# autonomousvision/LaRa

Hardware: AMD Instinct MI355X
Metric: novel-view frames/sec @512x512 (4-view in, 2DGS fwd+bwd) (higher is better)
Workload: dtype f32 raster + bf16-MFMA/f32-accumulate encoder (+ bf16-autocast coarse decoder MLP, as the reference's bf16-mixed)

## Files before the change

### lara_amd/csrc/group_attn.h

```cpp
#pragma once
#include "mfma_gemm.h"

namespace {


__device__ __forceinline__ float wave_total(float x) {
    x += dpp_move<0xB1, 0xf>(x);
    x += dpp_move<0x4E, 0xf>(x);
    x += dpp_move<0x141, 0xf>(x);
    x += dpp_move<0x140, 0xf>(x);
    x += dpp_move<0x142, 0xa>(x);
    x += dpp_move<0x143, 0xc>(x);
    return __int_as_float(__builtin_amdgcn_readlane(__float_as_int(x), 63));
}


__global__ void __launch_bounds__(256) pack_weight_frag_kernel(const unsigned short *__restrict__ W0, unsigned short *__restrict__ out0,
                                                               const unsigned short *__restrict__ W1, unsigned short *__restrict__ out1) {
    const bool second = blockIdx.x >= 32;
    const unsigned short *W = second ? W1 : W0;
    unsigned short *out = second ? out1 : out0;
    const int t = (blockIdx.x & 31) * 256 + threadIdx.x;
    const int lane = t & 63, ks = (t >> 6) & 15, nt = t >> 10;
    *(uint4 *)(out + (size_t)t * 8) = *(const uint4 *)(W + (size_t)(nt * 32 + (lane & 31)) * 256 + ks * 16 + 8 * (lane >> 5));
}

template <bool KEEP>
__global__ void __launch_bounds__(64)
group_attn_fused2_kernel(const float *x , const float *__restrict__ gamma,
                        const float *__restrict__ beta, const float eps, const unsigned short *__restrict__ Wq ,
                        const unsigned short *__restrict__ KV, const unsigned short *__restrict__ Wo , float *y, const int G,
                        unsigned short *__restrict__ xn_out, unsigned short *__restrict__ q_out, unsigned short *__restrict__ o_out) {
    constexpr int GA_LDS = 24576;
    __shared__ __attribute__((aligned(16))) unsigned char lds_all[GA_LDS];
    const int lane = threadIdx.x & 63;
    const int unit = blockIdx.x, g0 = unit * 4;
    if (g0 >= G) return;
    unsigned char *R = lds_all, *KVr = R + 16384;
    const int c16 = lane & 15, q4 = lane >> 4;
    const int q_rows = min(32, (G - g0) * 8), kv_rows = min(16, (G - g0) * 4);
    const int srow = lane >> 4, sphys = lane & 15;
    const size_t row0 = (size_t)g0 * 8;

    {
        const float4 gm = ((const float4 *)gamma)[lane], bt = ((const float4 *)beta)[lane];
        const int hh = lane >> 5, chunk = (lane & 31) >> 1, sub = (lane & 1) * 8;
#pragma unroll 1
        for (int rb = 0; rb < 32; rb += 16) {
            float4 v[16];
#pragma unroll
            for (int i = 0; i < 16; i++) v[i] = ((const float4 *)(x + (row0 + min(rb + i, q_rows - 1)) * 256))[lane];
#pragma unroll
            for (int i = 0; i < 16; i++) {
                const int r = rb + i;
                const float mean = wave_total((v[i].x + v[i].y) + (v[i].z + v[i].w)) * (1.0f / 256.0f);
                const float a = v[i].x - mean, b = v[i].y - mean, c = v[i].z - mean, d4 = v[i].w - mean;
                const float rstd = 1.0f / sqrtf(wave_total(a * a + b * b + c * c + d4 * d4) * (1.0f / 256.0f) + eps);
                *(uint2 *)(R + hh * 8192 + r * 256 + ((chunk ^ (r & 15)) << 4) + sub) =
                    make_uint2(f2bf2(a * rstd * gm.x + bt.x, b * rstd * gm.y + bt.y), f2bf2(c * rstd * gm.z + bt.z, d4 * rstd * gm.w + bt.w));
            }
        }
    }
    const int frow = lane & 31, fk = 8 * (lane >> 5);
    auto load_rows = [&](bf16x8 (&bf)[16]) {
#pragma unroll
        for (int ks = 0; ks < 16; ks++) {
            const int f = ks * 16 + fk;
            bf[ks] = *(const bf16x8 *)(R + (f >> 7) * 8192 + frow * 256 + ((((f & 127) >> 3) ^ (frow & 15)) << 4));
        }
    };
#pragma unroll
    for (int i = 0; i < 4; i++) {
        const int row = 4 * i + srow, chunk = sphys ^ (row & 15);
        const unsigned short *src = KV + (size_t)(g0 * 4 + min(row, kv_rows - 1)) * 512 + chunk * 8;
        __builtin_amdgcn_global_load_lds((const __attribute__((address_space(1))) void *)src,
                                         (__attribute__((address_space(3))) void *)(KVr + i * 1024), 16, 0, 0);
        __builtin_amdgcn_global_load_lds((const __attribute__((address_space(1))) void *)(src + 256),
                                         (__attribute__((address_space(3))) void *)(KVr + 4096 + i * 1024), 16, 0, 0);
    }
    auto store_rows = [&](unsigned short *dst) {
        asm volatile("s_waitcnt lgkmcnt(0)" ::: "memory");
#pragma unroll 4
        for (int i = 0; i < 16; i++) {
            const int r = 2 * i + (lane >> 5), c = lane & 31;
            const uint4 v = *(const uint4 *)(R + (c >> 4) * 8192 + r * 256 + (((c & 15) ^ (r & 15)) << 4));
            if (r < q_rows) *(uint4 *)(dst + (row0 + r) * 256 + c * 8) = v;
        }
    };
    bf16x8 bf[16], wf[16];
    load_rows(bf);
    if (KEEP) store_rows(xn_out);
#pragma unroll
    for (int ks = 0; ks < 16; ks++) wf[ks] = *(const bf16x8 *)(Wq + ((size_t)ks * 64 + lane) * 8);
#pragma unroll 1
    for (int nt = 0; nt < 8; nt++) {
        const unsigned short *wnext = Wq + ((size_t)min(nt + 1, 7) * 1024 + lane) * 8;
        bf16x8 wn[16];
#pragma unroll
        for (int ks = 0; ks < 16; ks++) wn[ks] = *(const bf16x8 *)(wnext + ks * 512);
        f32x16 acc;
#pragma unroll
        for (int i = 0; i < 16; i++) acc[i] = 0.f;
#pragma unroll
        for (int ks = 0; ks < 16; ks++) acc = __builtin_amdgcn_mfma_f32_32x32x16_bf16(wf[ks], bf[ks], acc, 0, 0, 0);
#pragma unroll
        for (int g = 0; g < 4; g++) {
            const int f = nt * 32 + 8 * g + 4 * (lane >> 5);
            *(uint2 *)(R + (f >> 7) * 8192 + frow * 256 + ((((f & 127) >> 3) ^ (frow & 15)) << 4) + ((f & 7) << 1)) =
                make_uint2(f2bf2(acc[4 * g], acc[4 * g + 1]), f2bf2(acc[4 * g + 2], acc[4 * g + 3]));
        }
#pragma unroll
        for (int ks = 0; ks < 16; ks++) wf[ks] = wn[ks];
    }
    if (KEEP) store_rows(q_out);
    asm volatile("s_waitcnt vmcnt(0)" ::: "memory");
    uint4 pk[4], pv[4];
#pragma unroll
    for (int i = 0; i < 4; i++) {
        const int row = 4 * i + srow, chunk = sphys ^ (row & 15);
        const unsigned short *src = KV + (size_t)(g0 * 4 + min(row, kv_rows - 1)) * 512 + 128 + chunk * 8;
        pk[i] = *(const uint4 *)src;
        pv[i] = *(const uint4 *)(src + 256);
    }
    for (int hh = 0; hh < 2; hh++) {
        unsigned char *Qr = R + hh * 8192, *Kr = KVr, *Vr = KVr + 4096;
        asm volatile("s_waitcnt lgkmcnt(0)" ::: "memory");
        if (hh == 1) {
#pragma unroll
            for (int i = 0; i < 4; i++) {
                *(uint4 *)(Kr + i * 1024 + lane * 16) = pk[i];
                *(uint4 *)(Vr + i * 1024 + lane * 16) = pv[i];
            }
            asm volatile("s_waitcnt lgkmcnt(0)" ::: "memory");
        }
#pragma unroll 2
        for (int hl = 0; hl < 8; hl++) {
            const int ck = 2 * hl + (q4 >> 1), sub = (q4 & 1) * 8;
            const s16x4 kf = *(const s16x4 *)(Kr + c16 * 256 + ((ck ^ c16) << 4) + sub);
            s16x4 vf;
            const int cv = 2 * hl + (c16 >> 3), vb = (c16 & 7) * 2;
#pragma unroll
            for (int e = 0; e < 4; e++) {
                const int row = 4 * q4 + e;
                vf[e] = *(const short *)(Vr + row * 256 + ((cv ^ row) << 4) + vb);
            }
#pragma unroll
            for (int t = 0; t < 2; t++) {
                const int qrow = 16 * t + c16;
                const s16x4 qf = *(const s16x4 *)(Qr + qrow * 256 + ((ck ^ (qrow & 15)) << 4) + sub);
                f32x4 sc = {0.f, 0.f, 0.f, 0.f};
                sc = __builtin_amdgcn_mfma_f32_16x16x16bf16_1k(kf, qf, sc, 0, 0, 0);
                const bool valid = q4 == 2 * t + (c16 >> 3);
                const float s0 = sc[0] * 0.25f, s1 = sc[1] * 0.25f, s2 = sc[2] * 0.25f, s3 = sc[3] * 0.25f;
                const float mx = fmaxf(fmaxf(s0, s1), fmaxf(s2, s3));
                const float e0 = __expf(s0 - mx), e1 = __expf(s1 - mx), e2 = __expf(s2 - mx), e3 = __expf(s3 - mx);
                const float inv = valid ? 1.0f / (e0 + e1 + e2 + e3) : 0.f;
                const uint2 pp = make_uint2(f2bf2(e0 * inv, e1 * inv), f2bf2(e2 * inv, e3 * inv));
                s16x4 pf;
                __builtin_memcpy(&pf, &pp, 8);
                f32x4 o = {0.f, 0.f, 0.f, 0.f};
                o = __builtin_amdgcn_mfma_f32_16x16x16bf16_1k(pf, vf, o, 0, 0, 0);
                const unsigned o01 = f2bf2(o[0], o[1]), o23 = f2bf2(o[2], o[3]);
#pragma unroll
                for (int rr = 0; rr < 4; rr++) {
                    const int orow = 16 * t + 4 * q4 + rr;
                    const unsigned w = rr < 2 ? o01 : o23;
                    *(unsigned short *)(Qr + orow * 256 + ((cv ^ (orow & 15)) << 4) + vb) = (unsigned short)((rr & 1) ? (w >> 16) : w);
                }
            }
        }
    }
    asm volatile("s_waitcnt lgkmcnt(0)" ::: "memory");
    if (KEEP) store_rows(o_out);
    load_rows(bf);
#pragma unroll
    for (int ks = 0; ks < 16; ks++) wf[ks] = *(const bf16x8 *)(Wo + ((size_t)ks * 64 + lane) * 8);
    float *T = (float *)R;
    const int erow = lane >> 3, ec = (lane & 7) * 4;
    float4 xr[4], xn4[4];
#pragma unroll
    for (int p4 = 0; p4 < 4; p4++) xr[p4] = *(const float4 *)(x + (row0 + min(erow + 8 * p4, q_rows - 1)) * 256 + ec);
#pragma unroll 1
    for (int nt = 0; nt < 8; nt++) {
        const unsigned short *wnext = Wo + ((size_t)min(nt + 1, 7) * 1024 + lane) * 8;
        bf16x8 wn[16];
#pragma unroll
        for (int ks = 0; ks < 16; ks++) wn[ks] = *(const bf16x8 *)(wnext + ks * 512);
#pragma unroll
        for (int p4 = 0; p4 < 4; p4++) xn4[p4] = *(const float4 *)(x + (row0 + min(erow + 8 * p4, q_rows - 1)) * 256 + min(nt + 1, 7) * 32 + ec);
        f32x16 acc;
#pragma unroll
        for (int i = 0; i < 16; i++) acc[i] = 0.f;
#pragma unroll
        for (int ks = 0; ks < 16; ks++) acc = __builtin_amdgcn_mfma_f32_32x32x16_bf16(wf[ks], bf[ks], acc, 0, 0, 0);
#pragma unroll
        for (int g = 0; g < 4; g++)
            *(float4 *)(T + frow * 36 + 8 * g + 4 * (lane >> 5)) = make_float4(acc[4 * g], acc[4 * g + 1], acc[4 * g + 2], acc[4 * g + 3]);
#pragma unroll
        for (int p4 = 0; p4 < 4; p4++) {
            const int row = erow + 8 * p4;
            const float4 v = *(const float4 *)(T + row * 36 + ec);
            if (row < q_rows)
                *(float4 *)(y + (row0 + row) * 256 + nt * 32 + ec) = make_float4(v.x + xr[p4].x, v.y + xr[p4].y, v.z + xr[p4].z, v.w + xr[p4].w);
        }
#pragma unroll
        for (int ks = 0; ks < 16; ks++) wf[ks] = wn[ks];
#pragma unroll
        for (int p4 = 0; p4 < 4; p4++) xr[p4] = xn4[p4];
    }
}

}
```

Baseline: 985.4.

## Split attention KV staging into quarter-heads to shrink LDS and raise occupancy

Restructures the fused group-attention kernel so K/V are staged into LDS one quarter (64 columns) at a time instead of per half, which cuts the LDS footprint from 24KB to 20KB. It also sets launch_bounds min-blocks to 2 and switches the intermediate xn/q/o stores to nontemporal stores. The goal is more resident waves per CU and less cache pollution, at the cost of more register prefetch of K/V (six fragments held) and four attend passes with extra waits. It also adds compile-time GA_TIMING switches that fake loads for profiling, plus a separate probe entry point.

After: 978.1. Within noise of the previous version (-0.7%).

```diff
diff --git a/lara_amd/csrc/attn_probe.hip b/lara_amd/csrc/attn_probe.hip
--- /dev/null
+++ b/lara_amd/csrc/attn_probe.hip
@@ -0,0 +1,27 @@
+#include "mfma_gemm.h"
+#include "group_attn.h"
+
+extern "C" {
+
+int lara_attnprobe_step(int keep, int project, int G, int cond_dim, const float *x, const unsigned short *cond_bf16, const float *ln_w,
+                        const float *ln_b, float eps, const unsigned short *wq, const unsigned short *wkv, const unsigned short *wo,
+                        float *y, unsigned short *kv, unsigned short *xn, unsigned short *q, unsigned short *o, void *wpack, void *stream) {
+    hipStream_t s = (hipStream_t)stream;
+    if (G <= 0 || !x || !ln_w || !ln_b || !wq || !wo || !y || !kv || !wpack) return hipErrorInvalidValue;
+    if (keep && (!xn || !q || !o)) return hipErrorInvalidValue;
+    if (project) {
+        if (!cond_bf16 || !wkv || cond_dim <= 0 || cond_dim % 32) return hipErrorInvalidValue;
+        GemmP p{};
+        p.A = cond_bf16; p.W = wkv; p.C = kv; p.M = G * 4; p.N = 512; p.K = cond_dim;
+        const hipError_t e = launch_gemm_ring<0, 0>(p, s);
+        if (e != hipSuccess) return e;
+    }
+    unsigned short *wqp = (unsigned short *)wpack, *wop = wqp + 65536;
+    const hipError_t e = L2D_LAUNCH_ERR(s, pack_weight_frag_kernel, dim3(64), dim3(256), 0, wq, wqp, wo, wop);
+    if (e != hipSuccess) return e;
+    if (keep) return L2D_LAUNCH_ERR(s, group_attn_fused2_kernel<true>, dim3((G + 3) / 4), dim3(64), 0, x, ln_w, ln_b, eps, wqp, kv, wop, y, G, xn, q, o);
+    return L2D_LAUNCH_ERR(s, group_attn_fused2_kernel<false>, dim3((G + 3) / 4), dim3(64), 0, x, ln_w, ln_b, eps, wqp, kv, wop, y, G,
+                          (unsigned short *)nullptr, (unsigned short *)nullptr, (unsigned short *)nullptr);
+}
+
+}
diff --git a/lara_amd/csrc/group_attn.h b/lara_amd/csrc/group_attn.h
--- a/lara_amd/csrc/group_attn.h
+++ b/lara_amd/csrc/group_attn.h
@@ -25,13 +25,17 @@
     *(uint4 *)(out + (size_t)t * 8) = *(const uint4 *)(W + (size_t)(nt * 32 + (lane & 31)) * 256 + ks * 16 + 8 * (lane >> 5));
 }
 
+#ifndef GA_TIMING
+#define GA_TIMING 0
+#endif
 template <bool KEEP>
-__global__ void __launch_bounds__(64)
+__global__ void __launch_bounds__(64, 2)
 group_attn_fused2_kernel(const float *x , const float *__restrict__ gamma,
                         const float *__restrict__ beta, const float eps, const unsigned short *__restrict__ Wq ,
                         const unsigned short *__restrict__ KV, const unsigned short *__restrict__ Wo , float *y, const int G,
                         unsigned short *__restrict__ xn_out, unsigned short *__restrict__ q_out, unsigned short *__restrict__ o_out) {
-    constexpr int GA_LDS = 24576;
+    typedef unsigned u32x4 __attribute__((ext_vector_type(4)));
+    constexpr int GA_LDS = 20480;
     __shared__ __attribute__((aligned(16))) unsigned char lds_all[GA_LDS];
     const int lane = threadIdx.x & 63;
     const int unit = blockIdx.x, g0 = unit * 4;
@@ -41,6 +45,12 @@
     const int q_rows = min(32, (G - g0) * 8), kv_rows = min(16, (G - g0) * 4);
     const int srow = lane >> 4, sphys = lane & 15;
     const size_t row0 = (size_t)g0 * 8;
+    constexpr bool KEPT = KEEP && !(GA_TIMING & 32);
+    auto kv_off = [](const int r, const int c) { return (r >> 1) * 256 + (((((r & 1) << 3) + c) ^ (r >> 1)) << 4); };
+    auto kv_src = [&](const int qd, const int i) {
+        const int rv = 4 * i + srow, C = sphys ^ rv, r = 2 * rv + (C >> 3);
+        return KV + (size_t)(g0 * 4 + min(r, kv_rows - 1)) * 512 + qd * 64 + (C & 7) * 8;
+    };
 
     {
         const float4 gm = ((const float4 *)gamma)[lane], bt = ((const float4 *)beta)[lane];
@@ -49,7 +59,15 @@
         for (int rb = 0; rb < 32; rb += 16) {
             float4 v[16];
 #pragma unroll
-            for (int i = 0; i < 16; i++) v[i] = ((const float4 *)(x + (row0 + min(rb + i, q_rows - 1)) * 256))[lane];
+            for (int i = 0; i < 16; i++) {
+                if (GA_TIMING & 1) {
+                    float4 t = make_float4((float)lane, (float)(lane >> 1), (float)(lane & 7), 1.f);
+                    asm volatile("" : "+v"(t.x), "+v"(t.y), "+v"(t.z), "+v"(t.w));
+                    v[i] = t;
+                } else {
+                    v[i] = ((const float4 *)(x + (row0 + min(rb + i, q_rows - 1)) * 256))[lane];
+                }
+            }
 #pragma unroll
             for (int i = 0; i < 16; i++) {
                 const int r = rb + i;
@@ -69,35 +87,46 @@
             bf[ks] = *(const bf16x8 *)(R + (f >> 7) * 8192 + frow * 256 + ((((f & 127) >> 3) ^ (frow & 15)) << 4));
         }
     };
-#pragma unroll
-    for (int i = 0; i < 4; i++) {
-        const int row = 4 * i + srow, chunk = sphys ^ (row & 15);
-        const unsigned short *src = KV + (size_t)(g0 * 4 + min(row, kv_rows - 1)) * 512 + chunk * 8;
-        __builtin_amdgcn_global_load_lds((const __attribute__((address_space(1))) void *)src,
-                                         (__attribute__((address_space(3))) void *)(KVr + i * 1024), 16, 0, 0);
-        __builtin_amdgcn_global_load_lds((const __attribute__((address_space(1))) void *)(src + 256),
-                                         (__attribute__((address_space(3))) void *)(KVr + 4096 + i * 1024), 16, 0, 0);
+    if (!(GA_TIMING & 4)) {
+#pragma unroll
+        for (int i = 0; i < 2; i++) {
+            const unsigned short *src = kv_src(0, i);
+            __builtin_amdgcn_global_load_lds((const __attribute__((address_space(1))) void *)src,
+                                             (__attribute__((address_space(3))) void *)(KVr + i * 1024), 16, 0, 0);
+            __builtin_amdgcn_global_load_lds((const __attribute__((address_space(1))) void *)(src + 256),
+                                             (__attribute__((address_space(3))) void *)(KVr + 2048 + i * 1024), 16, 0, 0);
+        }
     }
     auto store_rows = [&](unsigned short *dst) {
         asm volatile("s_waitcnt lgkmcnt(0)" ::: "memory");
 #pragma unroll 4
         for (int i = 0; i < 16; i++) {
             const int r = 2 * i + (lane >> 5), c = lane & 31;
-            const uint4 v = *(const uint4 *)(R + (c >> 4) * 8192 + r * 256 + (((c & 15) ^ (r & 15)) << 4));
-            if (r < q_rows) *(uint4 *)(dst + (row0 + r) * 256 + c * 8) = v;
-        }
-    };
+            const u32x4 v = *(const u32x4 *)(R + (c >> 4) * 8192 + r * 256 + (((c & 15) ^ (r & 15)) << 4));
+            if (r < q_rows) __builtin_nontemporal_store(v, (u32x4 *)(dst + (row0 + r) * 256 + c * 8));
+        }
+    };
+    auto wfrag = [&](const unsigned short *W, const int nt, const int ks, const bool fake) {
+        if (fake) {
+            const unsigned u = 0x3c003c00u + lane + ks;
+            const u32x4 t = {u, u + 1, u + 2, u + 3};
+            bf16x8 r;
+            __builtin_memcpy(&r, &t, 16);
+            return r;
+        }
+        return *(const bf16x8 *)(W + ((size_t)(nt * 16 + ks) * 64 + lane) * 8);
+    };
+    constexpr bool FQ = GA_TIMING & 2, FO = GA_TIMING & 8;
     bf16x8 bf[16], wf[16];
     load_rows(bf);
-    if (KEEP) store_rows(xn_out);
-#pragma unroll
-    for (int ks = 0; ks < 16; ks++) wf[ks] = *(const bf16x8 *)(Wq + ((size_t)ks * 64 + lane) * 8);
+    if (KEPT) store_rows(xn_out);
+#pragma unroll
+    for (int ks = 0; ks < 16; ks++) wf[ks] = wfrag(Wq, 0, ks, FQ);
 #pragma unroll 1
     for (int nt = 0; nt < 8; nt++) {
-        const unsigned short *wnext = Wq + ((size_t)min(nt + 1, 7) * 1024 + lane) * 8;
         bf16x8 wn[16];
 #pragma unroll
-        for (int ks = 0; ks < 16; ks++) wn[ks] = *(const bf16x8 *)(wnext + ks * 512);
+        for (int ks = 0; ks < 16; ks++) wn[ks] = wfrag(Wq, min(nt + 1, 7), ks, FQ);
         f32x16 acc;
 #pragma unroll
         for (int i = 0; i < 16; i++) acc[i] = 0.f;
@@ -112,37 +141,46 @@
 #pragma unroll
         for (int ks = 0; ks < 16; ks++) wf[ks] = wn[ks];
     }
-    if (KEEP) store_rows(q_out);
+    if (KEPT) store_rows(q_out);
     asm volatile("s_waitcnt vmcnt(0)" ::: "memory");
-    uint4 pk[4], pv[4];
-#pragma unroll
-    for (int i = 0; i < 4; i++) {
-        const int row = 4 * i + srow, chunk = sphys ^ (row & 15);
-        const unsigned short *src = KV + (size_t)(g0 * 4 + min(row, kv_rows - 1)) * 512 + 128 + chunk * 8;
-        pk[i] = *(const uint4 *)src;
-        pv[i] = *(const uint4 *)(src + 256);
-    }
-    for (int hh = 0; hh < 2; hh++) {
-        unsigned char *Qr = R + hh * 8192, *Kr = KVr, *Vr = KVr + 4096;
+    u32x4 pk[6], pv[6];
+#pragma unroll
+    for (int qd = 1; qd < 4; qd++) {
+#pragma unroll
+        for (int i = 0; i < 2; i++) {
+            if (GA_TIMING & 4) {
+                pk[2 * (qd - 1) + i] = u32x4{(unsigned)lane, (unsigned)qd, (unsigned)i, 0x3c003c00u};
+                pv[2 * (qd - 1) + i] = u32x4{(unsigned)lane, (unsigned)i, (unsigned)qd, 0x3c003c00u};
+            } else {
+                const unsigned short *src = kv_src(qd, i);
+                pk[2 * (qd - 1) + i] = *(const u32x4 *)src;
+                pv[2 * (qd - 1) + i] = *(const u32x4 *)(src + 256);
+            }
+        }
+    }
+    auto attend = [&](auto qdc) __attribute__((always_inline)) {
+        constexpr int qd = decltype(qdc)::value;
+        unsigned char *Qr = R + (qd >> 1) * 8192, *Kr = KVr, *Vr = KVr + 2048;
         asm volatile("s_waitcnt lgkmcnt(0)" ::: "memory");
-        if (hh == 1) {
-#pragma unroll
-            for (int i = 0; i < 4; i++) {
-                *(uint4 *)(Kr + i * 1024 + lane * 16) = pk[i];
-                *(uint4 *)(Vr + i * 1024 + lane * 16) = pv[i];
+        if constexpr (qd > 0) {
+#pragma unroll
+            for (int i = 0; i < 2; i++) {
+                *(u32x4 *)(Kr + i * 1024 + lane * 16) = pk[2 * (qd - 1) + i];
+                *(u32x4 *)(Vr + i * 1024 + lane * 16) = pv[2 * (qd - 1) + i];
             }
             asm volatile("s_waitcnt lgkmcnt(0)" ::: "memory");
         }
 #pragma unroll 2
-        for (int hl = 0; hl < 8; hl++) {
+        for (int hp = 0; hp < 4; hp++) {
+            const int hl = (qd & 1) * 4 + hp;
             const int ck = 2 * hl + (q4 >> 1), sub = (q4 & 1) * 8;
-            const s16x4 kf = *(const s16x4 *)(Kr + c16 * 256 + ((ck ^ c16) << 4) + sub);
+            const s16x4 kf = *(const s16x4 *)(Kr + kv_off(c16, 2 * hp + (q4 >> 1)) + sub);
             s16x4 vf;
             const int cv = 2 * hl + (c16 >> 3), vb = (c16 & 7) * 2;
 #pragma unroll
             for (int e = 0; e < 4; e++) {
                 const int row = 4 * q4 + e;
-                vf[e] = *(const short *)(Vr + row * 256 + ((cv ^ row) << 4) + vb);
+                vf[e] = *(const short *)(Vr + kv_off(row, 2 * hp + (c16 >> 3)) + vb);
             }
 #pragma unroll
             for (int t = 0; t < 2; t++) {
@@ -169,25 +207,33 @@
                 }
             }
         }
-    }
+    };
+    attend(std::integral_constant<int, 0>{});
+    attend(std::integral_constant<int, 1>{});
+    attend(std::integral_constant<int, 2>{});
+    attend(std::integral_constant<int, 3>{});
     asm volatile("s_waitcnt lgkmcnt(0)" ::: "memory");
-    if (KEEP) store_rows(o_out);
+    if (KEPT) store_rows(o_out);
     load_rows(bf);
 #pragma unroll
-    for (int ks = 0; ks < 16; ks++) wf[ks] = *(const bf16x8 *)(Wo + ((size_t)ks * 64 + lane) * 8);
+    for (int ks = 0; ks < 16; ks++) wf[ks] = wfrag(Wo, 0, ks, FO);
     float *T = (float *)R;
     const int erow = lane >> 3, ec = (lane & 7) * 4;
+    auto x_res = [&](float4 (&xr)[4], const int nt) {
+#pragma unroll
+        for (int p4 = 0; p4 < 4; p4++) {
+            if (GA_TIMING & 16) xr[p4] = make_float4((float)lane, (float)p4, (float)nt, 1.f);
+            else xr[p4] = *(const float4 *)(x + (row0 + min(erow + 8 * p4, q_rows - 1)) * 256 + nt * 32 + ec);
+        }
+    };
     float4 xr[4], xn4[4];
-#pragma unroll
-    for (int p4 = 0; p4 < 4; p4++) xr[p4] = *(const float4 *)(x + (row0 + min(erow + 8 * p4, q_rows - 1)) * 256 + ec);
+    x_res(xr, 0);
 #pragma unroll 1
     for (int nt = 0; nt < 8; nt++) {
-        const unsigned short *wnext = Wo + ((size_t)min(nt + 1, 7) * 1024 + lane) * 8;
         bf16x8 wn[16];
 #pragma unroll
-        for (int ks = 0; ks < 16; ks++) wn[ks] = *(const bf16x8 *)(wnext + ks * 512);
-#pragma unroll
-        for (int p4 = 0; p4 < 4; p4++) xn4[p4] = *(const float4 *)(x + (row0 + min(erow + 8 * p4, q_rows - 1)) * 256 + min(nt + 1, 7) * 32 + ec);
+        for (int ks = 0; ks < 16; ks++) wn[ks] = wfrag(Wo, min(nt + 1, 7), ks, FO);
+        x_res(xn4, min(nt + 1, 7));
         f32x16 acc;
 #pragma unroll
         for (int i = 0; i < 16; i++) acc[i] = 0.f;
@@ -200,8 +246,9 @@
         for (int p4 = 0; p4 < 4; p4++) {
             const int row = erow + 8 * p4;
             const float4 v = *(const float4 *)(T + row * 36 + ec);
-            if (row < q_rows)
-                *(float4 *)(y + (row0 + row) * 256 + nt * 32 + ec) = make_float4(v.x + xr[p4].x, v.y + xr[p4].y, v.z + xr[p4].z, v.w + xr[p4].w);
+            const float4 o4 = make_float4(v.x + xr[p4].x, v.y + xr[p4].y, v.z + xr[p4].z, v.w + xr[p4].w);
+            if (GA_TIMING & 16) asm volatile("" ::"v"(o4.x), "v"(o4.y), "v"(o4.z), "v"(o4.w));
+            else if (row < q_rows) *(float4 *)(y + (row0 + row) * 256 + nt * 32 + ec) = o4;
         }
 #pragma unroll
         for (int ks = 0; ks < 16; ks++) wf[ks] = wn[ks];
```
